# askerlee/segtran

Measured on NVIDIA H100. Metric: voxels/sec fwd+bwd Segtran3d BraTS 112^3 bs=4 hot path, higher is better.
Workload: dtype tf32

## Files before the change

### segtran_b200/csrc/sx_common.cuh

```cuda
#pragma once
#include <cuda.h>
#include <cuda_bf16.h>
#include <cuda_runtime.h>
#include <stdint.h>
#include <stdio.h>

#include "../../include/segtran_b200.h"

void sx_set_error(const char* fmt, ...);

#define SX_CHECK_CUDA(expr)                                                                     \
  do {                                                                                          \
    cudaError_t _e = (expr);                                                                    \
    if (_e != cudaSuccess) {                                                                    \
      sx_set_error("%s:%d CUDA error %s: %s", __FILE__, __LINE__, cudaGetErrorName(_e),         \
                   cudaGetErrorString(_e));                                                     \
      return -2;                                                                                \
    }                                                                                           \
  } while (0)

#define SX_REQUIRE(cond, ...)                                                                   \
  do {                                                                                          \
    if (!(cond)) {                                                                              \
      sx_set_error(__VA_ARGS__);                                                                \
      return -1;                                                                                \
    }                                                                                           \
  } while (0)

static inline int sx_ceil_div(int64_t a, int64_t b) { return (int)((a + b - 1) / b); }

static int sm_count_cached() {
  static int n[64] = {0};
  int dev = 0;
  if (cudaGetDevice(&dev) != cudaSuccess || dev < 0 || dev >= 64) return 0;
  if (n[dev] == 0) {
    int v = 0;
    if (cudaDeviceGetAttribute(&v, cudaDevAttrMultiProcessorCount, dev) != cudaSuccess) return 0;
    n[dev] = v;
  }
  return n[dev];
}


namespace sx {

__device__ __forceinline__ uint32_t smem_u32(const void* p) {
  return static_cast<uint32_t>(__cvta_generic_to_shared(p));
}

__device__ __forceinline__ bool elect_one() {
  uint32_t pred = 0;
  asm volatile(
      "{\n\t.reg .pred P;\n\t"
      "elect.sync _|P, 0xffffffff;\n\t"
      "selp.b32 %0, 1, 0, P;\n\t}\n"
      : "=r"(pred));
  return pred != 0;
}

__device__ __forceinline__ void mbar_init(uint64_t* bar, uint32_t count) {
  asm volatile("mbarrier.init.shared::cta.b64 [%0], %1;" ::"r"(smem_u32(bar)), "r"(count));
}
__device__ __forceinline__ void fence_barrier_init() {
  asm volatile("fence.mbarrier_init.release.cluster;" ::: "memory");
}
__device__ __forceinline__ void mbar_expect_tx(uint64_t* bar, uint32_t bytes) {
  asm volatile("mbarrier.arrive.expect_tx.shared::cta.b64 _, [%0], %1;" ::"r"(smem_u32(bar)), "r"(bytes)
               : "memory");
}
__device__ __forceinline__ void mbar_arrive(uint64_t* bar) {
  asm volatile("mbarrier.arrive.shared::cta.b64 _, [%0];" ::"r"(smem_u32(bar)) : "memory");
}
#ifndef SX_MBAR_TIMEOUT_NS
#define SX_MBAR_TIMEOUT_NS 4000000000ull
#endif
__device__ __forceinline__ uint64_t globaltimer_ns() {
  uint64_t t;
  asm volatile("mov.u64 %0, %%globaltimer;" : "=l"(t));
  return t;
}
__device__ __forceinline__ void mbar_wait(uint64_t* bar, uint32_t parity) {
  uint32_t ok = 0;
  const uint32_t addr = smem_u32(bar);
  uint64_t t0 = 0;
  while (true) {
    asm volatile(
        "{\n\t.reg .pred p;\n\t"
        "mbarrier.try_wait.parity.shared::cta.b64 p, [%1], %2;\n\t"
        "selp.b32 %0, 1, 0, p;\n\t}\n"
        : "=r"(ok)
        : "r"(addr), "r"(parity)
        : "memory");
    if (ok) break;
    const uint64_t now = globaltimer_ns();
    if (t0 == 0) t0 = now;
    if (now - t0 > SX_MBAR_TIMEOUT_NS) __trap();
  }
}

__device__ __forceinline__ void tma_prefetch_desc(const CUtensorMap* m) {
  asm volatile("prefetch.tensormap [%0];" ::"l"(reinterpret_cast<uint64_t>(m)) : "memory");
}
constexpr uint64_t kEvictNormal = 0x1000000000000000ull;
constexpr uint64_t kEvictFirst = 0x12F0000000000000ull;
constexpr uint64_t kEvictLast = 0x14F0000000000000ull;
__device__ __forceinline__ void tma_load_4d(void* smem_dst, const CUtensorMap* m, uint64_t* bar, int c0, int c1,
                                            int c2, int c3, uint64_t policy) {
  asm volatile(
      "cp.async.bulk.tensor.4d.shared::cluster.global.mbarrier::complete_tx::bytes.L2::cache_hint "
      "[%0], [%1, {%3, %4, %5, %6}], [%2], %7;" ::"r"(smem_u32(smem_dst)),
      "l"(reinterpret_cast<uint64_t>(m)), "r"(smem_u32(bar)), "r"(c0), "r"(c1), "r"(c2), "r"(c3), "l"(policy)
      : "memory");
}

__device__ __forceinline__ uint64_t gmma_desc(uint32_t saddr, uint32_t lbo_bytes, uint32_t sbo_bytes) {
  uint64_t d = 0;
  d |= (uint64_t)((saddr >> 4) & 0x3FFF);
  d |= (uint64_t)((lbo_bytes >> 4) & 0x3FFF) << 16;
  d |= (uint64_t)((sbo_bytes >> 4) & 0x3FFF) << 32;
  d |= (uint64_t)1 << 62;
  return d;
}
__device__ __forceinline__ void wgmma_fence() { asm volatile("wgmma.fence.sync.aligned;" ::: "memory"); }
__device__ __forceinline__ void wgmma_commit() { asm volatile("wgmma.commit_group.sync.aligned;" ::: "memory"); }
template <int N>
__device__ __forceinline__ void wgmma_wait() {
  asm volatile("wgmma.wait_group.sync.aligned %0;" ::"n"(N) : "memory");
}
__device__ __forceinline__ void fence_proxy_async_smem() {
  asm volatile("fence.proxy.async.shared::cta;" ::: "memory");
}
__device__ __forceinline__ void acc_fence(float (&d)[64]) {
#pragma unroll
  for (int i = 0; i < 64; ++i) asm volatile("" : "+f"(d[i])::"memory");
}
__device__ __forceinline__ void wgmma_tf32(float (&d)[64], uint64_t da, uint64_t db, uint32_t accumulate) {
  asm volatile(
      "{\n\t.reg .pred p;\n\tsetp.ne.b32 p, %66, 0;\n\t"
      "wgmma.mma_async.sync.aligned.m64n128k8.f32.tf32.tf32 "
      "{%0, %1, %2, %3, %4, %5, %6, %7, %8, %9, %10, %11, %12, %13, %14, %15, %16, %17, %18, %19, %20, %21, %22, %23, %24, %25, %26, %27, %28, %29, %30, %31, %32, %33, %34, %35, %36, %37, %38, %39, %40, %41, %42, %43, %44, %45, %46, %47, %48, %49, %50, %51, %52, %53, %54, %55, %56, %57, %58, %59, %60, %61, %62, %63}, "
      "%64, %65, p, 1, 1;\n\t}\n"
      : "+f"(d[0]), "+f"(d[1]), "+f"(d[2]), "+f"(d[3]), "+f"(d[4]), "+f"(d[5]), "+f"(d[6]), "+f"(d[7]), "+f"(d[8]), "+f"(d[9]), "+f"(d[10]), "+f"(d[11]), "+f"(d[12]), "+f"(d[13]), "+f"(d[14]), "+f"(d[15]), "+f"(d[16]), "+f"(d[17]), "+f"(d[18]), "+f"(d[19]), "+f"(d[20]), "+f"(d[21]), "+f"(d[22]), "+f"(d[23]), "+f"(d[24]), "+f"(d[25]), "+f"(d[26]), "+f"(d[27]), "+f"(d[28]), "+f"(d[29]), "+f"(d[30]), "+f"(d[31]), "+f"(d[32]), "+f"(d[33]), "+f"(d[34]), "+f"(d[35]), "+f"(d[36]), "+f"(d[37]), "+f"(d[38]), "+f"(d[39]), "+f"(d[40]), "+f"(d[41]), "+f"(d[42]), "+f"(d[43]), "+f"(d[44]), "+f"(d[45]), "+f"(d[46]), "+f"(d[47]), "+f"(d[48]), "+f"(d[49]), "+f"(d[50]), "+f"(d[51]), "+f"(d[52]), "+f"(d[53]), "+f"(d[54]), "+f"(d[55]), "+f"(d[56]), "+f"(d[57]), "+f"(d[58]), "+f"(d[59]), "+f"(d[60]), "+f"(d[61]), "+f"(d[62]), "+f"(d[63])
      : "l"(da), "l"(db), "r"(accumulate));
}
template <int TA, int TB>
__device__ __forceinline__ void wgmma_bf16(float (&d)[64], uint64_t da, uint64_t db, uint32_t accumulate) {
  asm volatile(
      "{\n\t.reg .pred p;\n\tsetp.ne.b32 p, %66, 0;\n\t"
      "wgmma.mma_async.sync.aligned.m64n128k16.f32.bf16.bf16 "
      "{%0, %1, %2, %3, %4, %5, %6, %7, %8, %9, %10, %11, %12, %13, %14, %15, %16, %17, %18, %19, %20, %21, %22, %23, %24, %25, %26, %27, %28, %29, %30, %31, %32, %33, %34, %35, %36, %37, %38, %39, %40, %41, %42, %43, %44, %45, %46, %47, %48, %49, %50, %51, %52, %53, %54, %55, %56, %57, %58, %59, %60, %61, %62, %63}, "
      "%64, %65, p, 1, 1, %67, %68;\n\t}\n"
      : "+f"(d[0]), "+f"(d[1]), "+f"(d[2]), "+f"(d[3]), "+f"(d[4]), "+f"(d[5]), "+f"(d[6]), "+f"(d[7]), "+f"(d[8]), "+f"(d[9]), "+f"(d[10]), "+f"(d[11]), "+f"(d[12]), "+f"(d[13]), "+f"(d[14]), "+f"(d[15]), "+f"(d[16]), "+f"(d[17]), "+f"(d[18]), "+f"(d[19]), "+f"(d[20]), "+f"(d[21]), "+f"(d[22]), "+f"(d[23]), "+f"(d[24]), "+f"(d[25]), "+f"(d[26]), "+f"(d[27]), "+f"(d[28]), "+f"(d[29]), "+f"(d[30]), "+f"(d[31]), "+f"(d[32]), "+f"(d[33]), "+f"(d[34]), "+f"(d[35]), "+f"(d[36]), "+f"(d[37]), "+f"(d[38]), "+f"(d[39]), "+f"(d[40]), "+f"(d[41]), "+f"(d[42]), "+f"(d[43]), "+f"(d[44]), "+f"(d[45]), "+f"(d[46]), "+f"(d[47]), "+f"(d[48]), "+f"(d[49]), "+f"(d[50]), "+f"(d[51]), "+f"(d[52]), "+f"(d[53]), "+f"(d[54]), "+f"(d[55]), "+f"(d[56]), "+f"(d[57]), "+f"(d[58]), "+f"(d[59]), "+f"(d[60]), "+f"(d[61]), "+f"(d[62]), "+f"(d[63])
      : "l"(da), "l"(db), "r"(accumulate), "n"(TA), "n"(TB));
}
__device__ __forceinline__ float round_tf32(float x) {
  uint32_t r;
  asm("cvt.rna.tf32.f32 %0, %1;" : "=r"(r) : "f"(x));
  return __uint_as_float(r);
}
__device__ __forceinline__ float ex2_approx(float x) {
  float y;
  asm("ex2.approx.ftz.f32 %0, %1;" : "=f"(y) : "f"(x));
  return y;
}
__device__ __forceinline__ float erf_fast(float x) {
  const float t = fminf(fabsf(x), 3.93f);
  float r = 4.5856195356464013e-05f;
  r = fmaf(r, t, -4.4942606473341584e-04f);
  r = fmaf(r, t, 1.5015227254480124e-03f);
  r = fmaf(r, t, 7.559903897345066e-04f);
  r = fmaf(r, t, -2.8238432481884956e-02f);
  r = fmaf(r, t, 1.4847517013549805e-01f);
  r = fmaf(r, t, 9.184176325798035e-01f);
  r = fmaf(r, t, 1.62790846824646f);
  const float y = 1.0f - ex2_approx(-r * t);
  return copysignf(y, x);
}
__device__ __forceinline__ float gelu_erf(float x) { return 0.5f * x * (1.0f + erf_fast(x * 0.70710678118654752f)); }
__device__ __forceinline__ float gelu_erf_grad(float x) {
  return 0.5f * (1.0f + erf_fast(x * 0.70710678118654752f)) + x * 0.3989422804014327f * __expf(-0.5f * x * x);
}
__device__ __forceinline__ uint32_t drop_p16(float p) {
  const float v = p * 65536.f + 0.5f;
  return v >= 65535.f ? 65535u : (uint32_t)v;
}
__device__ __forceinline__ uint32_t drop_mul(int w) { return w ? 0x85EBCA77u : 0x9E3779B1u; }
__device__ __forceinline__ uint32_t drop_key(unsigned long long seed, int w) {
  unsigned long long z = seed + (w ? 0x68E31DA4A0761D65ull : 0x9E3779B97F4A7C15ull);
  z = (z ^ (z >> 30)) * 0xBF58476D1CE4E5B9ull;
  z = (z ^ (z >> 27)) * 0x94D049BB133111EBull;
  z ^= z >> 31;
  return (uint32_t)z ^ (uint32_t)(z >> 32);
}
__device__ __forceinline__ uint32_t drop_word_k(uint32_t mul, uint32_t key, unsigned long long idx4) {
  uint32_t a = ((uint32_t)idx4 * mul) ^ key;
  a ^= (uint32_t)(idx4 >> 32) * 0xC2B2AE3Du;
  a ^= a >> 16; a *= 0x7FEB352Du; a ^= a >> 15; a *= 0x846CA68Bu; a ^= a >> 16;
  return a;
}
__device__ __forceinline__ uint2 drop_hash(unsigned long long seed, unsigned long long idx4) {
  return make_uint2(drop_word_k(drop_mul(0), drop_key(seed, 0), idx4), drop_word_k(drop_mul(1), drop_key(seed, 1), idx4));
}
__device__ __forceinline__ bool drop_keep(uint2 h, int j, uint32_t p16) {
  const uint32_t w = (j & 2) ? h.y : h.x;
  return ((w >> ((j & 1) * 16)) & 0xFFFFu) >= p16;
}
__device__ __forceinline__ bool drop_keep1(unsigned long long seed, unsigned long long idx, uint32_t p16) {
  const int j = (int)(idx & 3);
  const uint32_t w = drop_word_k(drop_mul(j >> 1), drop_key(seed, j >> 1), idx >> 2);
  return ((w >> ((j & 1) * 16)) & 0xFFFFu) >= p16;
}
__device__ __forceinline__ void atomic_max_float(float* addr, float v) {
  if (v >= 0.f)
    atomicMax(reinterpret_cast<int*>(addr), __float_as_int(v));
  else
    atomicMin(reinterpret_cast<unsigned int*>(addr), __float_as_uint(v));
}
__device__ __forceinline__ float warp_sum(float v) {
#pragma unroll
  for (int o = 16; o > 0; o >>= 1) v += __shfl_xor_sync(0xffffffffu, v, o);
  return v;
}
__device__ __forceinline__ float warp_max(float v) {
#pragma unroll
  for (int o = 16; o > 0; o >>= 1) v = fmaxf(v, __shfl_xor_sync(0xffffffffu, v, o));
  return v;
}

}
```

### segtran_b200/csrc/sx_gemm.cu

```cuda
#include <algorithm>
#include <string>

#include "sx_common.cuh"
#include "sx_tc.cuh"

namespace {
using namespace sxtc;

constexpr int NUM_THREADS = 384;
constexpr int STAGES = 4;
constexpr int STAGE_BYTES = A_STAGE_BYTES + B_STAGE_BYTES;
constexpr int XPOSE_WARPS = 3;

template <int ES, bool A_MN, bool B_MN>
struct Plan {
  static constexpr bool XA = ES == 4 && A_MN, XB = ES == 4 && B_MN;
  static constexpr bool XPOSE = XA || XB;
  static constexpr int RAW_BYTES = (XA ? A_STAGE_BYTES : 0) + (XB ? B_STAGE_BYTES : 0);
  static constexpr int RAW_SLOTS = !XPOSE ? 0 : (XA && XB ? 3 : 4);
  static constexpr int DIRECT_BYTES = STAGE_BYTES - RAW_BYTES;
  static constexpr int SMEM = STAGES * STAGE_BYTES + RAW_SLOTS * RAW_BYTES + 1024  + 256 ;
  static_assert(SMEM <= 227 * 1024, "sx_gemm: shared memory plan exceeds 227 KB");
  static_assert(!XPOSE || (A_STAGE_BYTES == 16384 && B_STAGE_BYTES == 16384 && BM == 128 && BN == 128),
                "sx_gemm: the transposer assumes 128-row, 16 KB tf32 operand tiles");
};

struct GemmParams {
  int M, N, K, Z0, Z1;
  int tiles_m, tiles_n, split_k, kb_per_split, num_kb, total_tiles;
  int z1_loop;
  float* part;
  int a_uses_z0, a_uses_z1, b_uses_z0, b_uses_z1;
  void* C;
  int c_bf16;
  int round_tf32;
  int c_vec_ok;
  long long ldc, c_sz0, c_sz1;
  float alpha;
  int bias_mode;
  const float* bias;
  long long bias_sz0, bias_sz1;
  int act;
  int accumulate;
  void* preact;
  float* amax;
  float drop_p;
  unsigned long long drop_seed;
  const unsigned long long* drop_seed_dev;
  const float* addend;
  int stream_out;
};

__device__ __forceinline__ void xpose_load(uint32_t src, int b, float4 (&v)[4]) {
  const int c = b & 7, kc = c ^ ((b >> 3) & 7);
  const uint32_t s = src + (b >> 6) * 4096;
#pragma unroll
  for (int e = 0; e < 4; ++e) {
    const int k = 4 * kc + e;
    asm volatile("ld.shared.v4.f32 {%0, %1, %2, %3}, [%4];"
                 : "=f"(v[e].x), "=f"(v[e].y), "=f"(v[e].z), "=f"(v[e].w)
                 : "r"(s + k * 128 + ((c ^ (k & 7)) << 4)) : "memory");
  }
}
__device__ __forceinline__ void xpose_store(uint32_t dst, int b, const float4 (&v)[4]) {
  const int c = b & 7, kc = c ^ ((b >> 3) & 7);
  const int r0 = (b >> 6) * 32 + 4 * c;
  auto st = [&](int i, float x, float y, float z, float w) {
    asm volatile("st.shared.v4.f32 [%0], {%1, %2, %3, %4};"
                 ::"r"(dst + (r0 + i) * 128 + ((kc ^ ((r0 + i) & 7)) << 4)), "f"(x), "f"(y), "f"(z), "f"(w) : "memory");
  };
  st(0, v[0].x, v[1].x, v[2].x, v[3].x);
  st(1, v[0].y, v[1].y, v[2].y, v[3].y);
  st(2, v[0].z, v[1].z, v[2].z, v[3].z);
  st(3, v[0].w, v[1].w, v[2].w, v[3].w);
}

template <int ES, bool A_MN, bool B_MN>
__global__ void __launch_bounds__(NUM_THREADS, 1)
sx_gemm_kernel(const __grid_constant__ CUtensorMap tmA, const __grid_constant__ CUtensorMap tmB, const GemmParams p) {
  using PL = Plan<ES, A_MN, B_MN>;
  constexpr bool kTF32 = (ES == 4);
  constexpr bool XA = PL::XA, XB = PL::XB;
  constexpr int BK = BKB / ES;
  constexpr int MN_BOX = BKB / ES;
  constexpr int MN_BOX_BYTES = BK * BKB;
  constexpr int KSTEPS = 4;

  extern __shared__ uint8_t smem_raw[];
  uint8_t* smem = reinterpret_cast<uint8_t*>((reinterpret_cast<uintptr_t>(smem_raw) + 1023) & ~uintptr_t(1023));
  uint8_t* raw = smem + STAGES * STAGE_BYTES;
  uint64_t* bars = reinterpret_cast<uint64_t*>(raw + PL::RAW_SLOTS * PL::RAW_BYTES);
  uint64_t* full_bar = bars;
  uint64_t* empty_bar = bars + STAGES;
  uint64_t* raw_full = bars + 2 * STAGES;
  uint64_t* raw_empty = raw_full + PL::RAW_SLOTS;

  const int warp = threadIdx.x >> 5;
  const int lane = threadIdx.x & 31;
  const int wg = threadIdx.x >> 7;

  if (threadIdx.x == 0) {
    sx::tma_prefetch_desc(&tmA);
    sx::tma_prefetch_desc(&tmB);
    for (int s = 0; s < STAGES; ++s) {
      sx::mbar_init(&full_bar[s], (PL::DIRECT_BYTES ? 1 : 0) + (PL::XPOSE ? XPOSE_WARPS : 0));
      sx::mbar_init(&empty_bar[s], 2);
    }
    for (int s = 0; s < PL::RAW_SLOTS; ++s) {
      sx::mbar_init(&raw_full[s], 1);
      sx::mbar_init(&raw_empty[s], XPOSE_WARPS);
    }
    sx::fence_barrier_init();
  }
  __syncthreads();

  auto decode = [&](int t, int& z0, int& z1, int& mb, int& nb, int& ks) {
    nb = t % p.tiles_n; t /= p.tiles_n;
    mb = t % p.tiles_m; t /= p.tiles_m;
    ks = t % p.split_k; t /= p.split_k;
    z0 = t % p.Z0;
    z1 = t / p.Z0;
  };
  auto split_kbs = [&](int ks) { return min(p.num_kb, (ks + 1) * p.kb_per_split) - ks * p.kb_per_split; };

  if (wg == 0) {
    asm volatile("setmaxnreg.dec.sync.aligned.u32 56;" ::: "memory");
    if (warp == 0) {
      if (sx::elect_one()) {
        int stage = 0, rs = 0;
        uint32_t phase = 0, rphase = 0;
        const uint64_t pol = p.stream_out ? sx::kEvictLast : sx::kEvictNormal;
        for (int t = blockIdx.x; t < p.total_tiles; t += gridDim.x) {
          int z0, z1, mb, nb, ks;
          decode(t, z0, z1, mb, nb, ks);
          const int kb0 = ks * p.kb_per_split;
          const int az0 = p.a_uses_z0 ? z0 : 0, bz0 = p.b_uses_z0 ? z0 : 0;
          const int m0 = mb * BM, n0 = nb * BN;
          const int nkb = split_kbs(ks);
          for (int q = 0; q < p.z1_loop * nkb; ++q) {
            const int kb = kb0 + q % nkb, zc = p.z1_loop > 1 ? q / nkb : z1;
            const int az1 = p.a_uses_z1 ? zc : 0, bz1 = p.b_uses_z1 ? zc : 0;
            const int k0 = kb * BK;
            if constexpr (PL::XPOSE) {
              sx::mbar_wait(&raw_empty[rs], rphase ^ 1);
              sx::mbar_expect_tx(&raw_full[rs], PL::RAW_BYTES);
              uint8_t* ra = raw + rs * PL::RAW_BYTES;
              uint8_t* rb = ra + (XA ? A_STAGE_BYTES : 0);
              if constexpr (XA) {
#pragma unroll
                for (int j = 0; j < BM / MN_BOX; ++j)
                  sx::tma_load_4d(ra + j * MN_BOX_BYTES, &tmA, &raw_full[rs], m0 + j * MN_BOX, k0, az0, az1, pol);
              }
              if constexpr (XB) {
#pragma unroll
                for (int j = 0; j < BN / MN_BOX; ++j)
                  sx::tma_load_4d(rb + j * MN_BOX_BYTES, &tmB, &raw_full[rs], n0 + j * MN_BOX, k0, bz0, bz1, pol);
              }
              if (++rs == PL::RAW_SLOTS) { rs = 0; rphase ^= 1; }
            }
            if constexpr (PL::DIRECT_BYTES > 0) {
              sx::mbar_wait(&empty_bar[stage], phase ^ 1);
              sx::mbar_expect_tx(&full_bar[stage], PL::DIRECT_BYTES);
              uint8_t* sa = smem + stage * STAGE_BYTES;
              uint8_t* sb = sa + A_STAGE_BYTES;
              if constexpr (!XA) {
                if constexpr (!A_MN) {
                  sx::tma_load_4d(sa, &tmA, &full_bar[stage], k0, m0, az0, az1, pol);
                } else {
#pragma unroll
                  for (int j = 0; j < BM / MN_BOX; ++j)
                    sx::tma_load_4d(sa + j * MN_BOX_BYTES, &tmA, &full_bar[stage], m0 + j * MN_BOX, k0, az0, az1, pol);
                }
              }
              if constexpr (!XB) {
                if constexpr (!B_MN) {
                  sx::tma_load_4d(sb, &tmB, &full_bar[stage], k0, n0, bz0, bz1, pol);
                } else {
#pragma unroll
                  for (int j = 0; j < BN / MN_BOX; ++j)
                    sx::tma_load_4d(sb + j * MN_BOX_BYTES, &tmB, &full_bar[stage], n0 + j * MN_BOX, k0, bz0, bz1, pol);
                }
              }
            }
            if (++stage == STAGES) { stage = 0; phase ^= 1; }
          }
        }
      }
    } else if constexpr (PL::XPOSE) {
      constexpr int NT = XPOSE_WARPS * 32;
      constexpr int NBLK = (XA && XB ? 2 : 1) * 256;
      const int xt = threadIdx.x - 32;
      int stage = 0, rs = 0;
      uint32_t phase = 0, rphase = 0;
      for (int t = blockIdx.x; t < p.total_tiles; t += gridDim.x) {
        int z0, z1, mb, nb, ks;
        decode(t, z0, z1, mb, nb, ks);
        const int nq = p.z1_loop * split_kbs(ks);
        for (int q = 0; q < nq; ++q) {
          sx::mbar_wait(&raw_full[rs], rphase);
          sx::mbar_wait(&empty_bar[stage], phase ^ 1);
          const uint32_t src = sx::smem_u32(raw + rs * PL::RAW_BYTES);
          const uint32_t dst = sx::smem_u32(smem + stage * STAGE_BYTES + (XA ? 0 : A_STAGE_BYTES));
          for (int b = xt; b < NBLK; b += NT) {
            float4 v[4];
            xpose_load(src + (b >> 8) * A_STAGE_BYTES, b & 255, v);
            xpose_store(dst + (b >> 8) * A_STAGE_BYTES, b & 255, v);
          }
          sx::fence_proxy_async_smem();
          __syncwarp();
          if (lane == 0) {
            sx::mbar_arrive(&full_bar[stage]);
            sx::mbar_arrive(&raw_empty[rs]);
          }
          if (++rs == PL::RAW_SLOTS) { rs = 0; rphase ^= 1; }
          if (++stage == STAGES) { stage = 0; phase ^= 1; }
        }
      }
    }
    return;
  }

  asm volatile("setmaxnreg.inc.sync.aligned.u32 224;" ::: "memory");
  const int cw = wg - 1;
  const int wtid = threadIdx.x & 127;
  const int wq = warp & 3;
  const int tr = lane >> 2;
  const int tc = (lane & 3) * 2;
  float tmax = -3.0e38f;
  int stage = 0;
  uint32_t phase = 0;

  auto desc_a = [&](const uint8_t* base, int kk, bool mn) -> uint64_t {
    const uint32_t a = sx::smem_u32(base) + (uint32_t)(cw * 64 * BKB);
    return mn ? sx::gmma_desc(a + kk * 16 * BKB, MN_BOX_BYTES, 1024) : sx::gmma_desc(a + kk * 32, 16, 1024);
  };
  auto desc_b = [&](const uint8_t* base, int kk, bool mn) -> uint64_t {
    const uint32_t b = sx::smem_u32(base);
    return mn ? sx::gmma_desc(b + kk * 16 * BKB, MN_BOX_BYTES, 1024) : sx::gmma_desc(b + kk * 32, 16, 1024);
  };

  auto store_frag = [&](void* base, const float (&f)[16], long long zoff, int row0, int col0, bool atomic_add) {
#pragma unroll
    for (int h = 0; h < 2; ++h) {
      const int grow = row0 + 8 * h + tr;
      if (grow < p.M) {
        const long long roff_ = zoff + (long long)grow * p.ldc;
#pragma unroll
        for (int j = 0; j < 4; ++j) {
          const int col = col0 + 8 * j + tc;
          const float a = f[4 * j + 2 * h], b = f[4 * j + 2 * h + 1];
          if (col + 1 < p.N) {
            if (p.c_bf16) {
              __nv_bfloat162 hb = __floats2bfloat162_rn(a, b);
              __nv_bfloat16* o = reinterpret_cast<__nv_bfloat16*>(base) + roff_ + col;
              if (p.c_vec_ok) *reinterpret_cast<__nv_bfloat162*>(o) = hb;
              else { o[0] = hb.x; o[1] = hb.y; }
            } else {
              float* o = reinterpret_cast<float*>(base) + roff_ + col;
              if (atomic_add) { atomicAdd(o, a); atomicAdd(o + 1, b); }
              else if (p.c_vec_ok) {
                if (p.stream_out) __stcs(reinterpret_cast<float2*>(o), make_float2(a, b));
                else *reinterpret_cast<float2*>(o) = make_float2(a, b);
              }
              else { o[0] = a; o[1] = b; }
            }
          } else if (col < p.N) {
            if (p.c_bf16) reinterpret_cast<__nv_bfloat16*>(base)[roff_ + col] = __float2bfloat16_rn(a);
            else if (atomic_add) atomicAdd(reinterpret_cast<float*>(base) + roff_ + col, a);
            else reinterpret_cast<float*>(base)[roff_ + col] = a;
          }
        }
      }
    }
  };

  auto load_frag = [&](const float* base, float (&g)[16], long long zoff, int row0, int col0) {
#pragma unroll
    for (int h = 0; h < 2; ++h) {
      const int grow = row0 + 8 * h + tr;
      const float* ar = base + zoff + (long long)(grow < p.M ? grow : 0) * p.ldc;
#pragma unroll
      for (int j = 0; j < 4; ++j) {
        const int col = col0 + 8 * j + tc;
        const int i0 = 4 * j + 2 * h;
        if (grow < p.M && col + 1 < p.N && p.c_vec_ok) {
          const float2 v = *reinterpret_cast<const float2*>(ar + col);
          g[i0] = v.x; g[i0 + 1] = v.y;
        } else {
          g[i0] = (grow < p.M && col < p.N) ? ar[col] : 0.f;
          g[i0 + 1] = (grow < p.M && col + 1 < p.N) ? ar[col + 1] : 0.f;
        }
      }
    }
  };

  const float drop_scale = p.drop_p > 0.f ? 1.f / (1.f - p.drop_p) : 1.f;
  const uint32_t drop_p16v = sx::drop_p16(p.drop_p);
  const unsigned long long drop_seed = p.drop_p > 0.f ? p.drop_seed + (p.drop_seed_dev ? *p.drop_seed_dev : 0ull) : 0ull;
  const uint32_t drop_mul_t = sx::drop_mul((tc >> 1) & 1), drop_key_t = sx::drop_key(drop_seed, (tc >> 1) & 1);

  float acc[64];
  for (int t = blockIdx.x; t < p.total_tiles; t += gridDim.x) {
    int z0, z1, mb, nb, ks;
    decode(t, z0, z1, mb, nb, ks);
    const int nq = p.z1_loop * split_kbs(ks);

    int prev = -1;
    for (int q = 0; q < nq; ++q) {
      sx::mbar_wait(&full_bar[stage], phase);
      const uint8_t* sa = smem + stage * STAGE_BYTES;
      const uint8_t* sb = sa + A_STAGE_BYTES;
      sx::acc_fence(acc);
      sx::wgmma_fence();
#pragma unroll
      for (int kk = 0; kk < KSTEPS; ++kk) {
        const uint64_t da = desc_a(sa, kk, A_MN && !kTF32), db = desc_b(sb, kk, B_MN && !kTF32);
        const uint32_t accum = (q > 0 || kk > 0) ? 1u : 0u;
        if constexpr (kTF32) sx::wgmma_tf32(acc, da, db, accum);
        else sx::wgmma_bf16<A_MN ? 1 : 0, B_MN ? 1 : 0>(acc, da, db, accum);
      }
      sx::wgmma_commit();
      sx::acc_fence(acc);
      sx::wgmma_wait<1>();
      if (prev >= 0 && wtid == 0) sx::mbar_arrive(&empty_bar[prev]);
      prev = stage;
      if (++stage == STAGES) { stage = 0; phase ^= 1; }
    }
    sx::wgmma_wait<0>();
    sx::acc_fence(acc);
    if (prev >= 0 && wtid == 0) sx::mbar_arrive(&empty_bar[prev]);

    const long long zoff = (long long)z1 * p.c_sz1 + (long long)z0 * p.c_sz0;
    const float* bias = p.bias ? p.bias + (long long)z1 * p.bias_sz1 + (long long)z0 * p.bias_sz0 : nullptr;
    const bool add_bias = (bias != nullptr) && (ks == 0);
    const int row0 = mb * BM + cw * 64 + wq * 16;
    float bias_m[2] = {0.f, 0.f};
    if (add_bias && p.bias_mode == SX_BIAS_M) {
#pragma unroll
      for (int h = 0; h < 2; ++h) {
        const int r = row0 + 8 * h + tr;
        bias_m[h] = r < p.M ? bias[r] : 0.f;
      }
    }
#pragma unroll
    for (int c = 0; c < BN / 32; ++c) {
      const int col0 = nb * BN + c * 32;
      if (col0 >= p.N) break;
      float f[16];
#pragma unroll
      for (int i = 0; i < 16; ++i) f[i] = acc[16 * c + i] * p.alpha + bias_m[(i >> 1) & 1];
      if (p.addend) {
        float g[16];
        load_frag(p.addend, g, zoff, row0, col0);
#pragma unroll
        for (int i = 0; i < 16; ++i) f[i] += g[i];
      }
      if (add_bias && p.bias_mode == SX_BIAS_N) {
#pragma unroll
        for (int j = 0; j < 4; ++j) {
          const int col = col0 + 8 * j + tc;
          const float b0 = col < p.N ? bias[col] : 0.f, b1 = col + 1 < p.N ? bias[col + 1] : 0.f;
#pragma unroll
          for (int h = 0; h < 2; ++h) {
            f[4 * j + 2 * h] += b0;
            f[4 * j + 2 * h + 1] += b1;
          }
        }
      }
      auto apply_dropout = [&]() {
        if (p.drop_p > 0.f) {
          if (((p.ldc | zoff) & 3) == 0) {
#pragma unroll
            for (int h = 0; h < 2; ++h) {
              const unsigned long long g0 =
                  (unsigned long long)((zoff + (long long)(row0 + 8 * h + tr) * p.ldc + col0 + tc) >> 2);
#pragma unroll
              for (int j = 0; j < 4; ++j) {
                const uint32_t bits = sx::drop_word_k(drop_mul_t, drop_key_t, g0 + 2 * j);
                const int i0 = 4 * j + 2 * h;
                f[i0] = (bits & 0xFFFFu) >= drop_p16v ? f[i0] * drop_scale : 0.f;
                f[i0 + 1] = (bits >> 16) >= drop_p16v ? f[i0 + 1] * drop_scale : 0.f;
              }
            }
          } else {
#pragma unroll
            for (int h = 0; h < 2; ++h) {
              const long long rbase = zoff + (long long)(row0 + 8 * h + tr) * p.ldc;
#pragma unroll
              for (int j = 0; j < 4; ++j) {
                const unsigned long long e0 = (unsigned long long)(rbase + col0 + 8 * j + tc);
                const int i0 = 4 * j + 2 * h;
                f[i0] = sx::drop_keep1(drop_seed, e0, drop_p16v) ? f[i0] * drop_scale : 0.f;
                f[i0 + 1] = sx::drop_keep1(drop_seed, e0 + 1, drop_p16v) ? f[i0 + 1] * drop_scale : 0.f;
              }
            }
          }
        }
      };
      if (p.act == SX_ACT_GELU_BWD) {
        apply_dropout();
        float g[16];
        load_frag(reinterpret_cast<const float*>(p.preact), g, zoff, row0, col0);
#pragma unroll
        for (int i = 0; i < 16; ++i) f[i] *= sx::gelu_erf_grad(g[i]);
      } else {
        if (p.preact) store_frag(p.preact, f, zoff, row0, col0, false);
        if (p.act == SX_ACT_GELU) {
#pragma unroll
          for (int i = 0; i < 16; ++i) f[i] = sx::gelu_erf(f[i]);
        }
        apply_dropout();
      }
      if (p.round_tf32 && !p.c_bf16) {
#pragma unroll
        for (int i = 0; i < 16; ++i) f[i] = sx::round_tf32(f[i]);
      }
      if (p.amax) {
#pragma unroll
        for (int h = 0; h < 2; ++h)
          if (row0 + 8 * h + tr < p.M) {
#pragma unroll
            for (int j = 0; j < 4; ++j)
#pragma unroll
              for (int e = 0; e < 2; ++e)
                if (col0 + 8 * j + tc + e < p.N) tmax = fmaxf(tmax, f[4 * j + 2 * h + e]);
          }
      }
      if (p.split_k > 1) {
        float* pt = p.part + ((((long long)z1 * p.Z0 + z0) * p.tiles_m + mb) * p.tiles_n + nb) * p.split_k * (BM * BN) +
                    (long long)ks * (BM * BN);
#pragma unroll
        for (int h = 0; h < 2; ++h)
#pragma unroll
          for (int j = 0; j < 4; ++j)
            *reinterpret_cast<float2*>(pt + (row0 - mb * BM + 8 * h + tr) * BN + (col0 - nb * BN) + 8 * j + tc) =
                make_float2(f[4 * j + 2 * h], f[4 * j + 2 * h + 1]);
      } else {
        store_frag(p.C, f, zoff, row0, col0, p.accumulate != 0);
      }
    }
  }
  if (p.amax) {
    tmax = sx::warp_max(tmax);
    if (lane == 0 && tmax > -3.0e38f) sx::atomic_max_float(p.amax, tmax);
  }
}

__global__ void split_reduce_kernel(const GemmParams p) {
  const long long total = (long long)p.total_tiles / p.split_k * (BM * BN);
  for (long long i = (long long)blockIdx.x * blockDim.x + threadIdx.x; i < total; i += (long long)gridDim.x * blockDim.x) {
    const int e = (int)(i % (BM * BN));
    long long t = i / (BM * BN);
    const int nb = (int)(t % p.tiles_n); t /= p.tiles_n;
    const int mb = (int)(t % p.tiles_m); t /= p.tiles_m;
    const int z0 = (int)(t % p.Z0), z1 = (int)(t / p.Z0);
    const int row = mb * BM + e / BN, col = nb * BN + e % BN;
    if (row >= p.M || col >= p.N) continue;
    const float* pt = p.part + (i / (BM * BN)) * p.split_k * (BM * BN) + e;
    float s = 0.f;
    for (int ks = 0; ks < p.split_k; ++ks) s += pt[(long long)ks * (BM * BN)];
    reinterpret_cast<float*>(p.C)[(long long)z1 * p.c_sz1 + (long long)z0 * p.c_sz0 + (long long)row * p.ldc + col] += s;
  }
}

long long g_max_ctas = -1;

template <int ES, bool A_MN, bool B_MN>
int launch(const CUtensorMap& ta, const CUtensorMap& tb, const GemmParams& p, int grid, cudaStream_t st) {
  auto kern = sx_gemm_kernel<ES, A_MN, B_MN>;
  constexpr int bytes = Plan<ES, A_MN, B_MN>::SMEM;
  SX_CHECK_CUDA(set_max_smem_once(kern, bytes));
  kern<<<grid, NUM_THREADS, bytes, st>>>(ta, tb, p);
  SX_CHECK_CUDA(cudaGetLastError());
  if (p.split_k > 1) {
    const long long n = (long long)p.total_tiles / p.split_k * (BM * BN);
    split_reduce_kernel<<<(int)std::min<long long>(sx_ceil_div(n, 256), 65535), 256, 0, st>>>(p);
    SX_CHECK_CUDA(cudaGetLastError());
  }
  return 0;
}

}

extern "C" int sx_gemm_debug_set(const char* key, int64_t value) {
  std::string k(key);
  if (k == "max_ctas") g_max_ctas = value;
  else {
    sx_set_error("sx_gemm_debug_set: unknown key %s", key);
    return -1;
  }
  return 0;
}

extern "C" int sx_gemm(const sx_gemm_args* a, void* stream) {
  SX_REQUIRE(a != nullptr, "sx_gemm: null args");
  SX_REQUIRE(a->M > 0 && a->N > 0 && a->K > 0 && a->Z0 > 0 && a->Z1 > 0, "sx_gemm: bad shape M=%d N=%d K=%d Z=%dx%d",
             a->M, a->N, a->K, a->Z0, a->Z1);
  SX_REQUIRE(a->op_dtype == SX_OP_TF32 || a->op_dtype == SX_OP_BF16, "sx_gemm: bad op_dtype %d", a->op_dtype);
  SX_REQUIRE(a->C != nullptr && a->A.ptr != nullptr && a->B.ptr != nullptr, "sx_gemm: null pointer");
  const int es = a->op_dtype == SX_OP_TF32 ? 4 : 2;
  const int bk = BKB / es;
  const int sms = sm_count_cached();
  SX_REQUIRE(sms > 0, "sx_gemm: no CUDA device (this library has no CPU fallback)");

  GemmParams p{};
  p.M = a->M; p.N = a->N; p.K = a->K; p.Z0 = a->Z0; p.Z1 = a->Z1;
  p.tiles_m = sx_ceil_div(a->M, BM);
  p.tiles_n = sx_ceil_div(a->N, BN);
  p.num_kb = sx_ceil_div(a->K, bk);
  const bool fold_z1 = a->Z1 > 1 && a->c_stride_z1 == 0;
  SX_REQUIRE(!fold_z1 || (a->accumulate && !a->bias && !a->addend && a->act == SX_ACT_NONE && !a->preact && a->drop_p == 0.f),
             "sx_gemm: a z1-reduced output needs accumulate=1 and a linear epilogue without bias");
  p.z1_loop = fold_z1 ? a->Z1 : 1;
  p.Z1 = fold_z1 ? 1 : a->Z1;
  int split = a->split_k < 1 ? 1 : a->split_k;
  if (split > p.num_kb) split = p.num_kb;
  {
    const long long out_tiles = (long long)p.tiles_m * p.tiles_n * a->Z0 * p.Z1;
    const long long fit = a->part ? a->part_floats / ((long long)BM * BN * out_tiles) : 0;
    if (split > fit) split = fit < 2 ? 1 : (int)fit;
  }
  p.kb_per_split = sx_ceil_div(p.num_kb, split);
  p.split_k = sx_ceil_div(p.num_kb, p.kb_per_split);
  SX_REQUIRE(p.split_k == 1 || (a->accumulate && a->c_dtype == SX_F32 && a->act == SX_ACT_NONE && !a->preact &&
                                a->drop_p == 0.f && !a->amax),
             "sx_gemm: split_k > 1 needs accumulate=1 into fp32 C and a linear epilogue");
  SX_REQUIRE(!a->accumulate || a->c_dtype == SX_F32, "sx_gemm: accumulate needs fp32 C");
  SX_REQUIRE(!a->round_tf32 || (!a->accumulate && p.split_k == 1),
             "sx_gemm: round_tf32 cannot be combined with accumulate / split_k > 1 (a sum of rounded partials is not a TF32 "
             "value): round the finished output instead");
  const long long tt = (long long)p.tiles_m * p.tiles_n * p.split_k * a->Z0 * p.Z1;
  SX_REQUIRE(tt < (1ll << 30), "sx_gemm: too many tiles");
  p.total_tiles = (int)tt;
  p.a_uses_z0 = a->A.stride_z0 != 0; p.a_uses_z1 = a->A.stride_z1 != 0;
  p.b_uses_z0 = a->B.stride_z0 != 0; p.b_uses_z1 = a->B.stride_z1 != 0;
  p.C = a->C; p.c_bf16 = a->c_dtype == SX_BF16; p.round_tf32 = a->round_tf32;
  p.ldc = a->ldc; p.c_sz0 = a->c_stride_z0; p.c_sz1 = a->c_stride_z1;
  p.c_vec_ok = ((reinterpret_cast<uintptr_t>(a->C) & 7) == 0) && (a->ldc % 2 == 0) && (a->c_stride_z0 % 2 == 0) &&
               (a->c_stride_z1 % 2 == 0) && (!a->preact || (reinterpret_cast<uintptr_t>(a->preact) & 7) == 0) &&
               (!a->addend || (reinterpret_cast<uintptr_t>(a->addend) & 7) == 0);
  p.alpha = a->alpha; p.bias_mode = a->bias ? a->bias_mode : SX_BIAS_NONE; p.bias = a->bias;
  p.bias_sz0 = a->bias_stride_z0; p.bias_sz1 = a->bias_stride_z1;
  p.act = a->act; p.accumulate = a->accumulate; p.preact = a->preact; p.amax = a->amax;
  p.addend = a->addend;
  SX_REQUIRE(a->act != SX_ACT_GELU_BWD || (a->preact && a->c_dtype == SX_F32 && p.split_k == 1 && !a->accumulate),
             "sx_gemm: SX_ACT_GELU_BWD needs the fp32 pre-activation in `preact`, fp32 C, split_k=1, accumulate=0");
  SX_REQUIRE(!a->addend || (p.split_k == 1 && !a->accumulate && a->c_dtype == SX_F32), "sx_gemm: addend needs split_k=1, accumulate=0, fp32 C");
  p.drop_p = a->drop_p; p.drop_seed = a->drop_seed;
  p.drop_seed_dev = reinterpret_cast<const unsigned long long*>(a->drop_seed_dev);
  {
    const double out_bytes = (double)a->M * a->N * a->Z0 * a->Z1 * (p.c_bf16 ? 2 : 4) * (a->preact ? 2 : 1);
    p.stream_out = out_bytes > 25.0 * 1024 * 1024;
  }

  CUtensorMap ta, tb;
  int rc = make_map(&ta, a->A, es, a->M, a->K, a->Z0, a->Z1, BM, "A");
  if (rc) return rc;
  rc = make_map(&tb, a->B, es, a->N, a->K, a->Z0, a->Z1, BN, "B");
  if (rc) return rc;

  int grid = p.total_tiles < sms ? p.total_tiles : sms;
  if (g_max_ctas > 0 && grid > g_max_ctas) grid = (int)g_max_ctas;
  p.part = a->part;
  cudaStream_t st = reinterpret_cast<cudaStream_t>(stream);
  const bool amn = a->A.major == SX_MAJOR_MN, bmn = a->B.major == SX_MAJOR_MN;
  if (es == 4) {
    if (!amn && !bmn) return launch<4, false, false>(ta, tb, p, grid, st);
    if (!amn && bmn) return launch<4, false, true>(ta, tb, p, grid, st);
    if (amn && !bmn) return launch<4, true, false>(ta, tb, p, grid, st);
    return launch<4, true, true>(ta, tb, p, grid, st);
  }
  if (!amn && !bmn) return launch<2, false, false>(ta, tb, p, grid, st);
  if (!amn && bmn) return launch<2, false, true>(ta, tb, p, grid, st);
  if (amn && !bmn) return launch<2, true, false>(ta, tb, p, grid, st);
  return launch<2, true, true>(ta, tb, p, grid, st);
}
```

Baseline: 461.6 million.

## Add 128x256 tf32 GEMM tile variant using m64n256k8 wgmma

```diff
diff --git a/segtran_b200/csrc/sx_common.cuh b/segtran_b200/csrc/sx_common.cuh
--- a/segtran_b200/csrc/sx_common.cuh
+++ b/segtran_b200/csrc/sx_common.cuh
@@ -130,9 +130,10 @@
 __device__ __forceinline__ void fence_proxy_async_smem() {
   asm volatile("fence.proxy.async.shared::cta;" ::: "memory");
 }
-__device__ __forceinline__ void acc_fence(float (&d)[64]) {
+template <int N>
+__device__ __forceinline__ void acc_fence(float (&d)[N]) {
 #pragma unroll
-  for (int i = 0; i < 64; ++i) asm volatile("" : "+f"(d[i])::"memory");
+  for (int i = 0; i < N; ++i) asm volatile("" : "+f"(d[i])::"memory");
 }
 __device__ __forceinline__ void wgmma_tf32(float (&d)[64], uint64_t da, uint64_t db, uint32_t accumulate) {
   asm volatile(
@@ -141,6 +142,15 @@
       "{%0, %1, %2, %3, %4, %5, %6, %7, %8, %9, %10, %11, %12, %13, %14, %15, %16, %17, %18, %19, %20, %21, %22, %23, %24, %25, %26, %27, %28, %29, %30, %31, %32, %33, %34, %35, %36, %37, %38, %39, %40, %41, %42, %43, %44, %45, %46, %47, %48, %49, %50, %51, %52, %53, %54, %55, %56, %57, %58, %59, %60, %61, %62, %63}, "
       "%64, %65, p, 1, 1;\n\t}\n"
       : "+f"(d[0]), "+f"(d[1]), "+f"(d[2]), "+f"(d[3]), "+f"(d[4]), "+f"(d[5]), "+f"(d[6]), "+f"(d[7]), "+f"(d[8]), "+f"(d[9]), "+f"(d[10]), "+f"(d[11]), "+f"(d[12]), "+f"(d[13]), "+f"(d[14]), "+f"(d[15]), "+f"(d[16]), "+f"(d[17]), "+f"(d[18]), "+f"(d[19]), "+f"(d[20]), "+f"(d[21]), "+f"(d[22]), "+f"(d[23]), "+f"(d[24]), "+f"(d[25]), "+f"(d[26]), "+f"(d[27]), "+f"(d[28]), "+f"(d[29]), "+f"(d[30]), "+f"(d[31]), "+f"(d[32]), "+f"(d[33]), "+f"(d[34]), "+f"(d[35]), "+f"(d[36]), "+f"(d[37]), "+f"(d[38]), "+f"(d[39]), "+f"(d[40]), "+f"(d[41]), "+f"(d[42]), "+f"(d[43]), "+f"(d[44]), "+f"(d[45]), "+f"(d[46]), "+f"(d[47]), "+f"(d[48]), "+f"(d[49]), "+f"(d[50]), "+f"(d[51]), "+f"(d[52]), "+f"(d[53]), "+f"(d[54]), "+f"(d[55]), "+f"(d[56]), "+f"(d[57]), "+f"(d[58]), "+f"(d[59]), "+f"(d[60]), "+f"(d[61]), "+f"(d[62]), "+f"(d[63])
+      : "l"(da), "l"(db), "r"(accumulate));
+}
+__device__ __forceinline__ void wgmma_tf32_n256(float (&d)[128], uint64_t da, uint64_t db, uint32_t accumulate) {
+  asm volatile(
+      "{\n\t.reg .pred p;\n\tsetp.ne.b32 p, %130, 0;\n\t"
+      "wgmma.mma_async.sync.aligned.m64n256k8.f32.tf32.tf32 "
+      "{%0, %1, %2, %3, %4, %5, %6, %7, %8, %9, %10, %11, %12, %13, %14, %15, %16, %17, %18, %19, %20, %21, %22, %23, %24, %25, %26, %27, %28, %29, %30, %31, %32, %33, %34, %35, %36, %37, %38, %39, %40, %41, %42, %43, %44, %45, %46, %47, %48, %49, %50, %51, %52, %53, %54, %55, %56, %57, %58, %59, %60, %61, %62, %63, %64, %65, %66, %67, %68, %69, %70, %71, %72, %73, %74, %75, %76, %77, %78, %79, %80, %81, %82, %83, %84, %85, %86, %87, %88, %89, %90, %91, %92, %93, %94, %95, %96, %97, %98, %99, %100, %101, %102, %103, %104, %105, %106, %107, %108, %109, %110, %111, %112, %113, %114, %115, %116, %117, %118, %119, %120, %121, %122, %123, %124, %125, %126, %127}, "
+      "%128, %129, p, 1, 1;\n\t}\n"
+      : "+f"(d[0]), "+f"(d[1]), "+f"(d[2]), "+f"(d[3]), "+f"(d[4]), "+f"(d[5]), "+f"(d[6]), "+f"(d[7]), "+f"(d[8]), "+f"(d[9]), "+f"(d[10]), "+f"(d[11]), "+f"(d[12]), "+f"(d[13]), "+f"(d[14]), "+f"(d[15]), "+f"(d[16]), "+f"(d[17]), "+f"(d[18]), "+f"(d[19]), "+f"(d[20]), "+f"(d[21]), "+f"(d[22]), "+f"(d[23]), "+f"(d[24]), "+f"(d[25]), "+f"(d[26]), "+f"(d[27]), "+f"(d[28]), "+f"(d[29]), "+f"(d[30]), "+f"(d[31]), "+f"(d[32]), "+f"(d[33]), "+f"(d[34]), "+f"(d[35]), "+f"(d[36]), "+f"(d[37]), "+f"(d[38]), "+f"(d[39]), "+f"(d[40]), "+f"(d[41]), "+f"(d[42]), "+f"(d[43]), "+f"(d[44]), "+f"(d[45]), "+f"(d[46]), "+f"(d[47]), "+f"(d[48]), "+f"(d[49]), "+f"(d[50]), "+f"(d[51]), "+f"(d[52]), "+f"(d[53]), "+f"(d[54]), "+f"(d[55]), "+f"(d[56]), "+f"(d[57]), "+f"(d[58]), "+f"(d[59]), "+f"(d[60]), "+f"(d[61]), "+f"(d[62]), "+f"(d[63]), "+f"(d[64]), "+f"(d[65]), "+f"(d[66]), "+f"(d[67]), "+f"(d[68]), "+f"(d[69]), "+f"(d[70]), "+f"(d[71]), "+f"(d[72]), "+f"(d[73]), "+f"(d[74]), "+f"(d[75]), "+f"(d[76]), "+f"(d[77]), "+f"(d[78]), "+f"(d[79]), "+f"(d[80]), "+f"(d[81]), "+f"(d[82]), "+f"(d[83]), "+f"(d[84]), "+f"(d[85]), "+f"(d[86]), "+f"(d[87]), "+f"(d[88]), "+f"(d[89]), "+f"(d[90]), "+f"(d[91]), "+f"(d[92]), "+f"(d[93]), "+f"(d[94]), "+f"(d[95]), "+f"(d[96]), "+f"(d[97]), "+f"(d[98]), "+f"(d[99]), "+f"(d[100]), "+f"(d[101]), "+f"(d[102]), "+f"(d[103]), "+f"(d[104]), "+f"(d[105]), "+f"(d[106]), "+f"(d[107]), "+f"(d[108]), "+f"(d[109]), "+f"(d[110]), "+f"(d[111]), "+f"(d[112]), "+f"(d[113]), "+f"(d[114]), "+f"(d[115]), "+f"(d[116]), "+f"(d[117]), "+f"(d[118]), "+f"(d[119]), "+f"(d[120]), "+f"(d[121]), "+f"(d[122]), "+f"(d[123]), "+f"(d[124]), "+f"(d[125]), "+f"(d[126]), "+f"(d[127])
       : "l"(da), "l"(db), "r"(accumulate));
 }
 template <int TA, int TB>
diff --git a/segtran_b200/csrc/sx_gemm.cu b/segtran_b200/csrc/sx_gemm.cu
--- a/segtran_b200/csrc/sx_gemm.cu
+++ b/segtran_b200/csrc/sx_gemm.cu
@@ -9,11 +9,15 @@
 
 constexpr int NUM_THREADS = 384;
 constexpr int STAGES = 4;
-constexpr int STAGE_BYTES = A_STAGE_BYTES + B_STAGE_BYTES;
 constexpr int XPOSE_WARPS = 3;
-
-template <int ES, bool A_MN, bool B_MN>
+constexpr int BN_WIDE = 256;
+
+template <int ES, bool A_MN, bool B_MN, int BN_T>
 struct Plan {
+  static_assert(BN_T == BN || (BN_T == BN_WIDE && ES == 4 && !A_MN && !B_MN),
+                "sx_gemm: the 256-column tile is instantiated for K-major tf32 operands only");
+  static constexpr int B_BYTES = BN_T * BKB;
+  static constexpr int STAGE_BYTES = A_STAGE_BYTES + B_BYTES;
   static constexpr bool XA = ES == 4 && A_MN, XB = ES == 4 && B_MN;
   static constexpr bool XPOSE = XA || XB;
   static constexpr int RAW_BYTES = (XA ? A_STAGE_BYTES : 0) + (XB ? B_STAGE_BYTES : 0);
@@ -75,11 +79,13 @@
   st(3, v[0].w, v[1].w, v[2].w, v[3].w);
 }
 
-template <int ES, bool A_MN, bool B_MN>
+template <int ES, bool A_MN, bool B_MN, int BN_T>
 __global__ void __launch_bounds__(NUM_THREADS, 1)
 sx_gemm_kernel(const __grid_constant__ CUtensorMap tmA, const __grid_constant__ CUtensorMap tmB, const GemmParams p) {
-  using PL = Plan<ES, A_MN, B_MN>;
+  using PL = Plan<ES, A_MN, B_MN, BN_T>;
   constexpr bool kTF32 = (ES == 4);
+  constexpr bool WIDE = BN_T == BN_WIDE;
+  constexpr int STAGE_BYTES = PL::STAGE_BYTES;
   constexpr bool XA = PL::XA, XB = PL::XB;
   constexpr int BK = BKB / ES;
   constexpr int MN_BOX = BKB / ES;
@@ -124,7 +130,8 @@
   auto split_kbs = [&](int ks) { return min(p.num_kb, (ks + 1) * p.kb_per_split) - ks * p.kb_per_split; };
 
   if (wg == 0) {
-    asm volatile("setmaxnreg.dec.sync.aligned.u32 56;" ::: "memory");
+    if constexpr (WIDE) asm volatile("setmaxnreg.dec.sync.aligned.u32 40;" ::: "memory");
+    else asm volatile("setmaxnreg.dec.sync.aligned.u32 56;" ::: "memory");
     if (warp == 0) {
       if (sx::elect_one()) {
         int stage = 0, rs = 0;
@@ -135,7 +142,7 @@
           decode(t, z0, z1, mb, nb, ks);
           const int kb0 = ks * p.kb_per_split;
           const int az0 = p.a_uses_z0 ? z0 : 0, bz0 = p.b_uses_z0 ? z0 : 0;
-          const int m0 = mb * BM, n0 = nb * BN;
+          const int m0 = mb * BM, n0 = nb * BN_T;
           const int nkb = split_kbs(ks);
           for (int q = 0; q < p.z1_loop * nkb; ++q) {
             const int kb = kb0 + q % nkb, zc = p.z1_loop > 1 ? q / nkb : z1;
@@ -153,7 +160,7 @@
               }
               if constexpr (XB) {
 #pragma unroll
-                for (int j = 0; j < BN / MN_BOX; ++j)
+                for (int j = 0; j < BN_T / MN_BOX; ++j)
                   sx::tma_load_4d(rb + j * MN_BOX_BYTES, &tmB, &raw_full[rs], n0 + j * MN_BOX, k0, bz0, bz1, pol);
               }
               if (++rs == PL::RAW_SLOTS) { rs = 0; rphase ^= 1; }
@@ -177,7 +184,7 @@
                   sx::tma_load_4d(sb, &tmB, &full_bar[stage], k0, n0, bz0, bz1, pol);
                 } else {
 #pragma unroll
-                  for (int j = 0; j < BN / MN_BOX; ++j)
+                  for (int j = 0; j < BN_T / MN_BOX; ++j)
                     sx::tma_load_4d(sb + j * MN_BOX_BYTES, &tmB, &full_bar[stage], n0 + j * MN_BOX, k0, bz0, bz1, pol);
                 }
               }
@@ -220,13 +227,13 @@
     return;
   }
 
-  asm volatile("setmaxnreg.inc.sync.aligned.u32 224;" ::: "memory");
+  if constexpr (WIDE) asm volatile("setmaxnreg.inc.sync.aligned.u32 232;" ::: "memory");
+  else asm volatile("setmaxnreg.inc.sync.aligned.u32 224;" ::: "memory");
   const int cw = wg - 1;
   const int wtid = threadIdx.x & 127;
   const int wq = warp & 3;
   const int tr = lane >> 2;
   const int tc = (lane & 3) * 2;
-  float tmax = -3.0e38f;
   int stage = 0;
   uint32_t phase = 0;
 
@@ -299,7 +306,7 @@
   const unsigned long long drop_seed = p.drop_p > 0.f ? p.drop_seed + (p.drop_seed_dev ? *p.drop_seed_dev : 0ull) : 0ull;
   const uint32_t drop_mul_t = sx::drop_mul((tc >> 1) & 1), drop_key_t = sx::drop_key(drop_seed, (tc >> 1) & 1);
 
-  float acc[64];
+  float acc[BN_T / 2];
   for (int t = blockIdx.x; t < p.total_tiles; t += gridDim.x) {
     int z0, z1, mb, nb, ks;
     decode(t, z0, z1, mb, nb, ks);
@@ -316,7 +323,8 @@
       for (int kk = 0; kk < KSTEPS; ++kk) {
         const uint64_t da = desc_a(sa, kk, A_MN && !kTF32), db = desc_b(sb, kk, B_MN && !kTF32);
         const uint32_t accum = (q > 0 || kk > 0) ? 1u : 0u;
-        if constexpr (kTF32) sx::wgmma_tf32(acc, da, db, accum);
+        if constexpr (WIDE) sx::wgmma_tf32_n256(acc, da, db, accum);
+        else if constexpr (kTF32) sx::wgmma_tf32(acc, da, db, accum);
         else sx::wgmma_bf16<A_MN ? 1 : 0, B_MN ? 1 : 0>(acc, da, db, accum);
       }
       sx::wgmma_commit();
@@ -334,6 +342,7 @@
     const float* bias = p.bias ? p.bias + (long long)z1 * p.bias_sz1 + (long long)z0 * p.bias_sz0 : nullptr;
     const bool add_bias = (bias != nullptr) && (ks == 0);
     const int row0 = mb * BM + cw * 64 + wq * 16;
+    float tmax = -3.0e38f;
     float bias_m[2] = {0.f, 0.f};
     if (add_bias && p.bias_mode == SX_BIAS_M) {
 #pragma unroll
@@ -342,13 +351,14 @@
         bias_m[h] = r < p.M ? bias[r] : 0.f;
       }
     }
-#pragma unroll
-    for (int c = 0; c < BN / 32; ++c) {
-      const int col0 = nb * BN + c * 32;
+    constexpr int EPI_UNROLL = WIDE ? 1 : BN_T / 32;
+#pragma unroll EPI_UNROLL
+    for (int c = 0; c < BN_T / 32; ++c) {
+      const int col0 = nb * BN_T + c * 32;
       if (col0 >= p.N) break;
       float f[16];
 #pragma unroll
-      for (int i = 0; i < 16; ++i) f[i] = acc[16 * c + i] * p.alpha + bias_m[(i >> 1) & 1];
+      for (int i = 0; i < 16; ++i) f[i] = acc[(WIDE ? 0 : 16 * c) + i] * p.alpha + bias_m[(i >> 1) & 1];
       if (p.addend) {
         float g[16];
         load_frag(p.addend, g, zoff, row0, col0);
@@ -426,7 +436,7 @@
                 if (col0 + 8 * j + tc + e < p.N) tmax = fmaxf(tmax, f[4 * j + 2 * h + e]);
           }
       }
-      if (p.split_k > 1) {
+      if (!WIDE && p.split_k > 1) {
         float* pt = p.part + ((((long long)z1 * p.Z0 + z0) * p.tiles_m + mb) * p.tiles_n + nb) * p.split_k * (BM * BN) +
                     (long long)ks * (BM * BN);
 #pragma unroll
@@ -438,11 +448,15 @@
       } else {
         store_frag(p.C, f, zoff, row0, col0, p.accumulate != 0);
       }
-    }
-  }
-  if (p.amax) {
-    tmax = sx::warp_max(tmax);
-    if (lane == 0 && tmax > -3.0e38f) sx::atomic_max_float(p.amax, tmax);
+      if constexpr (WIDE) {
+#pragma unroll
+        for (int i = 0; i < BN_T / 2 - 16; ++i) acc[i] = acc[i + 16];
+      }
+    }
+    if (p.amax) {
+      tmax = sx::warp_max(tmax);
+      if (lane == 0 && tmax > -3.0e38f) sx::atomic_max_float(p.amax, tmax);
+    }
   }
 }
 
@@ -464,11 +478,12 @@
 }
 
 long long g_max_ctas = -1;
-
-template <int ES, bool A_MN, bool B_MN>
+int g_wide_tiles = -1;
+
+template <int ES, bool A_MN, bool B_MN, int BN_T = BN>
 int launch(const CUtensorMap& ta, const CUtensorMap& tb, const GemmParams& p, int grid, cudaStream_t st) {
-  auto kern = sx_gemm_kernel<ES, A_MN, B_MN>;
-  constexpr int bytes = Plan<ES, A_MN, B_MN>::SMEM;
+  auto kern = sx_gemm_kernel<ES, A_MN, B_MN, BN_T>;
+  constexpr int bytes = Plan<ES, A_MN, B_MN, BN_T>::SMEM;
   SX_CHECK_CUDA(set_max_smem_once(kern, bytes));
   kern<<<grid, NUM_THREADS, bytes, st>>>(ta, tb, p);
   SX_CHECK_CUDA(cudaGetLastError());
@@ -485,6 +500,7 @@
 extern "C" int sx_gemm_debug_set(const char* key, int64_t value) {
   std::string k(key);
   if (k == "max_ctas") g_max_ctas = value;
+  else if (k == "wide_tiles") g_wide_tiles = value < 0 ? -1 : (value ? 1 : 0);
   else {
     sx_set_error("sx_gemm_debug_set: unknown key %s", key);
     return -1;
@@ -529,6 +545,11 @@
   SX_REQUIRE(!a->round_tf32 || (!a->accumulate && p.split_k == 1),
              "sx_gemm: round_tf32 cannot be combined with accumulate / split_k > 1 (a sum of rounded partials is not a TF32 "
              "value): round the finished output instead");
+  const bool amn = a->A.major == SX_MAJOR_MN, bmn = a->B.major == SX_MAJOR_MN;
+  const bool wide_legal = es == 4 && !amn && !bmn && p.split_k == 1;
+  const long long wide_tt = (long long)p.tiles_m * sx_ceil_div(a->N, BN_WIDE) * a->Z0 * p.Z1;
+  const bool wide = wide_legal && (g_wide_tiles == 1 || (g_wide_tiles < 0 && a->N > BN && 2 * wide_tt > sms));
+  if (wide) p.tiles_n = sx_ceil_div(a->N, BN_WIDE);
   const long long tt = (long long)p.tiles_m * p.tiles_n * p.split_k * a->Z0 * p.Z1;
   SX_REQUIRE(tt < (1ll << 30), "sx_gemm: too many tiles");
   p.total_tiles = (int)tt;
@@ -556,14 +577,14 @@
   CUtensorMap ta, tb;
   int rc = make_map(&ta, a->A, es, a->M, a->K, a->Z0, a->Z1, BM, "A");
   if (rc) return rc;
-  rc = make_map(&tb, a->B, es, a->N, a->K, a->Z0, a->Z1, BN, "B");
+  rc = make_map(&tb, a->B, es, a->N, a->K, a->Z0, a->Z1, wide ? BN_WIDE : BN, "B");
   if (rc) return rc;
 
   int grid = p.total_tiles < sms ? p.total_tiles : sms;
   if (g_max_ctas > 0 && grid > g_max_ctas) grid = (int)g_max_ctas;
   p.part = a->part;
   cudaStream_t st = reinterpret_cast<cudaStream_t>(stream);
-  const bool amn = a->A.major == SX_MAJOR_MN, bmn = a->B.major == SX_MAJOR_MN;
+  if (wide) return launch<4, false, false, BN_WIDE>(ta, tb, p, grid, st);
   if (es == 4) {
     if (!amn && !bmn) return launch<4, false, false>(ta, tb, p, grid, st);
     if (!amn && bmn) return launch<4, false, true>(ta, tb, p, grid, st);
```

New measurement: 508.6 million, median of 6. 10.2% higher.
